# psc0628/NeRF-PRV

Hardware: AMD Instinct MI355X
Metric: ray-samples/s (field evaluations composited; candidate views rendered + scored; scene baseline, field 256^3) (higher is better)
Workload: dtype f16

## Files before the change

### nerf_prv_amd/csrc/prv_kernels.hip

```cpp
#include "prv_kernels.hpp"

#include <algorithm>

#ifndef PRV_ABLATE
#define PRV_ABLATE 0
#endif

namespace prv {


__device__ __forceinline__ void morton16(uint32_t i, uint32_t& x, uint32_t& y) {
  x = (i & 1u) | ((i >> 1) & 2u) | ((i >> 2) & 4u) | ((i >> 3) & 8u);
  y = ((i >> 1) & 1u) | ((i >> 2) & 2u) | ((i >> 3) & 4u) | ((i >> 4) & 8u);
}

constexpr float kNgpDt = 1.7320508075688772f / 1024.0f;

__device__ __forceinline__ uint32_t march_ngp(const FieldDev& fd, const float o[3], const float d[3], float t0, float t1,
                                              uint32_t (*mw)[256], int& k_lo, int& k_hi, int& first_nz, int& last_nz) {
  const float dt = kNgpDt;
  first_nz = 32;
  last_nz = -1;
  k_lo = k_hi = 0;
  float ta = t0, tb = t1;
// ... 483 lines not shown
    for (int e = 0; e < E; e++) {
      k2_lo = min(k2_lo, first_nz[e]);
      k2_hi = max(k2_hi, last_nz[e]);
    }
    uint32_t acc[E][4];
#pragma unroll
    for (int e = 0; e < E; e++)
#pragma unroll
      for (int q = 0; q < 4; q++) acc[e][q] = 0u;
    for (int k = k2_lo; k <= k2_hi; k++) {
      uint32_t w[E];
      bool behind = false;
#pragma unroll
      for (int e = 0; e < E; e++) behind = behind || (k - first_nz[e] >= kWin && k <= last_nz[e]);
      if (!((passmask >> k) & 1u)) {
#pragma unroll
        for (int e = 0; e < E; e++) w[e] = 0u;
      } else if (behind) {
        fine_word(k, w);
      } else {
#pragma unroll
        for (int e = 0; e < E; e++) {
          const int j = k - first_nz[e];
          w[e] = (j >= 0 && k <= last_nz[e]) ? mw[e][j][threadIdx.x] : 0u;
        }
      }
#pragma unroll
      for (int e = 0; e < E; e++) {
        const int j = k - first_nz[e];
        if (j < 0 || k > last_nz[e]) continue;
        const int q = j & 3;
        if (j < 4) {
#pragma unroll
          for (int u = 0; u < 4; u++)
            if (q == u) m[e][u] = w[e];
        } else {
#pragma unroll
          for (int u = 0; u < 4; u++)
            if (q == u) acc[e][u] = w[e];
          if ((q == 3 || k == last_nz[e]) && !(PRV_ABLATE & 128)) {
            const uint32_t slot = base[e] + (uint32_t)__popcll(b[e] & ((1ull << lane) - 1ull));
            P.mem[e].queue_ext[(size_t)((j >> 2) - 1) * ext_stride + slot] = make_uint4(acc[e][0], acc[e][1], acc[e][2], acc[e][3]);
#pragma unroll
            for (int u = 0; u < 4; u++) acc[e][u] = 0u;
          }
        }
      }
    }
  }
#pragma unroll
  for (int e = 0; e < E; e++) {
    const MarchSink Q{P.mem[e].queue, P.mem[e].queue_ext, ext_stride, P.mem[e].queue_count, P.mem[e].out_f32, P.mem[e].out_u8};
    march_write<true, true>(P, Q, stage, r, first_nz[e] < 32, b[e], base[e], dt, m[e], first_nz[e], last_nz[e], [](int) { return 0u; });
  }
}

__global__ __launch_bounds__(256) void occ_interleave_kernel(OccInterleaveParams P) {
  const uint32_t c = blockIdx.x * 256u + threadIdx.x;
  if (c >= P.n_cells) return;
  uint32_t v = 0u;
  for (int e = 0; e < P.n_members; e++) v |= ((P.bits[e][c >> 5] >> (c & 31u)) & 1u) << e;
  P.out[c] = (uint8_t)v;
}


__device__ __forceinline__ void clock_stamp_begin(unsigned long long* stat) {
  if (blockIdx.x == 0 && threadIdx.x == 0) {
    stat[4] = __builtin_readcyclecounter();
    stat[5] = __builtin_amdgcn_s_memrealtime();
  }
}
__device__ __forceinline__ void clock_stamp_end(unsigned long long* stat) {
  if (blockIdx.x == 0 && threadIdx.x == 0) {
    atomicAdd(stat + 2, __builtin_readcyclecounter() - stat[4]);
    atomicAdd(stat + 3, __builtin_amdgcn_s_memrealtime() - stat[5]);
  }
}

__device__ __forceinline__ int lane_id() { return (int)(threadIdx.x & 63u); }

__device__ __forceinline__ float entropy_add(float p, float H) { return p >= 1.17549435e-38f ? fmaf(p, -__builtin_amdgcn_logf(p), H) : H; }

enum : int { kRenderColour = 0, kRenderDepth = 1, kRenderEntropy = 2 };
template <int F, int NDENSE, bool NGP, bool CACHE, int MODE>
__device__ __forceinline__ void render_queue64_body(RenderParams P, const RenderDepthParams* PD, const RenderEntropyParams* PE = nullptr) {
  constexpr bool DEPTH = MODE == kRenderDepth, ENTROPY = MODE == kRenderEntropy;
  constexpr int kMoveWords = ENTROPY ? 4 : DEPTH ? 7 : 6;
  constexpr int kFrags = ENTROPY ? 8 : kNumFrags;
  __shared__ half8 wl[kFrags * 64];
  __shared__ uint32_t mv[4][32][kMoveWords];
  constexpr uint32_t kPoolCap = 192;
  __shared__ uint32_t pool[kPoolCap][kMoveWords];
  __shared__ uint32_t pool_n, pool_lock;
  for (int i = threadIdx.x; i < kFrags * 64; i += 256) wl[i] = P.field.frags64[i];
  if (threadIdx.x == 0) {
    pool_n = 0u;
    pool_lock = 0u;
  }
  __syncthreads();
  auto pool_acquire = [&]() {
    if (lane_id() == 0)
      while (atomicCAS(&pool_lock, 0u, 1u) != 0u) __builtin_amdgcn_s_sleep(2);
    __builtin_amdgcn_fence(__ATOMIC_ACQUIRE, "workgroup");
    __builtin_amdgcn_wave_barrier();
  };
  auto pool_release = [&]() {
    __builtin_amdgcn_fence(__ATOMIC_RELEASE, "workgroup");
    __builtin_amdgcn_wave_barrier();
    if (lane_id() == 0) atomicExch(&pool_lock, 0u);
  };
  const LevelDev* __restrict__ lvl = P.field.levels;
  const HashConsts hc = {P.field.hash_my_b, P.field.hash_mz_b, P.field.hash_m_b, (uint32_t)P.field.wide_offsets};

  const int lane = threadIdx.x & 63, r = lane & 31, g = lane >> 5;

  bool active = false;
  uint32_t pix = 0, rec_i = 0;
  float o[3] = {0, 0, 0}, d[3] = {0, 0, 1}, t0 = 0.f, dt = 0.f;
  uint32_t cur = 0, m1 = 0, m2 = 0, m3 = 0, base = 0;
  float T = 1.f, cr = 0.f, cg = 0.f, cb = 0.f;
  float D = 0.f;
  float Hs = 0.f;
  half8 shA = {0, 0, 0, 0, 0, 0, 0, 0}, shB = {0, 0, 0, 0, 0, 0, 0, 0};
  bool drained = false;
  unsigned long long n_eval = 0ull, n_rounds = 0ull;
  constexpr int kCached = CACHE ? 32 / F - NDENSE : 1;
  CornerCache<F> cc[kCached];
#pragma unroll
  for (int j = 0; j < kCached; j++) cc[j].key = ~0u;
  clock_stamp_begin(P.stat_evaluated);
  uint32_t q_cur = 0, q_end = 0;
  const uint32_t n_seg = (uint32_t)P.n_segments;
  const uint32_t n_sub = (uint32_t)max(P.n_sub, 1);
  uint32_t seg = n_seg > 1u ? (((uint32_t)__builtin_amdgcn_s_getreg((3 << 11) | 20) & 7u) % (n_seg / n_sub)) * n_sub + (blockIdx.x * 4u + (threadIdx.x >> 6)) % n_sub : 0u;
  uint32_t seg_tried = 0;
  const uint4* __restrict__ queue = reinterpret_cast<const uint4*>(P.queue);

  auto take_ray = [&](uint32_t ri, uint32_t next) {
    const uint4* rec = queue + (size_t)ri * kRecordWords;
    const uint4 q0 = rec[0], q1 = rec[1], q3 = rec[3];
    uint4 mk = rec[2];
    o[0] = __uint_as_float(q0.x); o[1] = __uint_as_float(q0.y); o[2] = __uint_as_float(q0.z);
    t0 = __uint_as_float(q0.w);
    d[0] = __uint_as_float(q1.x); d[1] = __uint_as_float(q1.y); d[2] = __uint_as_float(q1.z);
    dt = __uint_as_float(q1.w);
    pix = q3.x;
    rec_i = ri;
    base = 0u;
    if constexpr (NGP) {
      const uint32_t base0 = q3.y & 0xffffu;
      base = base0;
      if (next >= base0 + 128u) {
        const uint32_t j = (next - base0) >> 7;
        mk = P.queue_ext[(size_t)(j - 1u) * ((size_t)P.seg_cap * (size_t)P.n_segments) + (size_t)ri];
        base = base0 + 128u * j;
      }
    }
    cur = mk.x; m1 = mk.y; m2 = mk.z; m3 = mk.w;
    while (base + 32u <= next) {
      cur = m1; m1 = m2; m2 = m3; m3 = 0u;
      base += 32u;
    }
    if (next > base) cur &= ~0u << (next & 31u);
    while (cur == 0u && (m1 | m2 | m3) != 0u) {
      cur = m1; m1 = m2; m2 = m3; m3 = 0u;
      base += 32u;
    }
    active = true;
  };
  auto next_chunk = [&]() -> bool {
    const uint32_t info = queue[(size_t)rec_i * kRecordWords + 3].y;
    const uint32_t base0 = info & 0xffffu, n_chunks = info >> 16;
    for (uint32_t j = ((base - base0) >> 7) + 1u; j < n_chunks; j++) {
      const uint4 mk = P.queue_ext[(size_t)(j - 1u) * ((size_t)P.seg_cap * (size_t)P.n_segments) + (size_t)rec_i];
      if ((mk.x | mk.y | mk.z | mk.w) == 0u) continue;
      cur = mk.x; m1 = mk.y; m2 = mk.z; m3 = mk.w;
      base = base0 + 128u * j;
      while (cur == 0u) {
        cur = m1; m1 = m2; m2 = m3; m3 = 0u;
        base += 32u;
      }
      return true;
    }
    return false;
  };

  for (;;) {
    const bool relocate = (n_rounds & 6ull) == 0ull;
    if (relocate && !drained && P.merge_max > 0) {
      const unsigned long long act0 = __ballot(active);
      const uint32_t aA = (uint32_t)act0, aB = (uint32_t)(act0 >> 32);
      const uint32_t nA = (uint32_t)__popc(aA), nB = (uint32_t)__popc(aB);
      int src = -1;
      if (nA != 0u && nB != 0u) {
        if (nA <= (uint32_t)P.merge_max && nA <= 32u - nB) src = 0;
        else if (nB <= (uint32_t)P.merge_max && nB <= 32u - nA) src = 1;
      }
      if (src >= 0) {
        const uint32_t a_src = src == 0 ? aA : aB, a_dst = src == 0 ? aB : aA, n_src = src == 0 ? nA : nB;
        const uint32_t below = (1u << r) - 1u;
        uint32_t(*slot)[kMoveWords] = mv[threadIdx.x >> 6];
        if (g == src && active) {
          uint32_t* e = slot[__popc(a_src & below)];
          e[0] = rec_i;
          e[1] = base + (uint32_t)__builtin_ctz(cur);
          e[2] = __float_as_uint(T);
          if constexpr (ENTROPY) {
            e[3] = __float_as_uint(Hs);
          } else {
            e[3] = __float_as_uint(cr);
            e[4] = __float_as_uint(cg);
            e[5] = __float_as_uint(cb);
          }
          if constexpr (DEPTH) e[6] = __float_as_uint(D);
          active = false;
        }
        __builtin_amdgcn_fence(__ATOMIC_RELEASE, "wavefront");
        __builtin_amdgcn_wave_barrier();
        __builtin_amdgcn_fence(__ATOMIC_ACQUIRE, "wavefront");
        const uint32_t kth = (uint32_t)__popc(~a_dst & below);
        if (!((a_dst >> r) & 1u) && kth < n_src) {
          const uint32_t* e = slot[kth];
          const uint32_t ri = e[0];
          if constexpr (!ENTROPY) {
            const half8 sh = reinterpret_cast<const half8*>(queue + (size_t)ri * kRecordWords)[4 + g];
            if (src == 0) shB = sh;
            else shA = sh;
          }
          if (g != src) {
            T = __uint_as_float(e[2]);
            if constexpr (ENTROPY) {
              Hs = __uint_as_float(e[3]);
            } else {
              cr = __uint_as_float(e[3]); cg = __uint_as_float(e[4]); cb = __uint_as_float(e[5]);
            }
            if constexpr (DEPTH) D = __uint_as_float(e[6]);
            take_ray(ri, e[1]);
          }
        }
        __builtin_amdgcn_wave_barrier();
      }
    }
    if (P.pool_on && (relocate || drained)) {
      const unsigned long long act1 = __ballot(active);
      const uint32_t below = (1u << r) - 1u;
      const uint32_t in_pool = *(volatile uint32_t*)&pool_n;
#pragma unroll
      for (int grp = 0; grp < 2; grp++) {
        const uint32_t a_g = grp == 0 ? (uint32_t)act1 : (uint32_t)(act1 >> 32), n_g = (uint32_t)__popc(a_g);
        if (!drained && n_g != 0u && n_g <= (uint32_t)P.merge_max && in_pool + n_g <= kPoolCap) {
          pool_acquire();
          const uint32_t at = *(volatile uint32_t*)&pool_n;
          const bool fits = at + n_g <= kPoolCap;
          if (fits && g == grp && active) {
            uint32_t* e = pool[at + (uint32_t)__popc(a_g & below)];
            e[0] = rec_i;
            e[1] = base + (uint32_t)__builtin_ctz(cur);
            e[2] = __float_as_uint(T);
            if constexpr (ENTROPY) {
              e[3] = __float_as_uint(Hs);
            } else {
              e[3] = __float_as_uint(cr);
              e[4] = __float_as_uint(cg);
              e[5] = __float_as_uint(cb);
            }
            if constexpr (DEPTH) e[6] = __float_as_uint(D);
            active = false;
          }
          if (fits && lane == 0) *(volatile uint32_t*)&pool_n = at + n_g;
          pool_release();
        }
      }
      const unsigned long long act2 = __ballot(active);
#pragma unroll
      for (int grp = 0; grp < 2; grp++) {
        const uint32_t a_g = grp == 0 ? (uint32_t)act2 : (uint32_t)(act2 >> 32);
        const uint32_t n_idle = 32u - (uint32_t)__popc(a_g);
        if (n_idle == 0u || (a_g == 0u && !drained) || *(volatile uint32_t*)&pool_n == 0u) continue;
        pool_acquire();
        const uint32_t have = *(volatile uint32_t*)&pool_n;
        const uint32_t take = min(have, n_idle), from = have - take;
        const uint32_t kth = (uint32_t)__popc(~a_g & below);
        uint32_t ent[kMoveWords] = {};
        const bool mine = !((a_g >> r) & 1u) && kth < take;
        if (mine) {
#pragma unroll
          for (int q = 0; q < kMoveWords; q++) ent[q] = pool[from + kth][q];
        }
        if (lane == 0) *(volatile uint32_t*)&pool_n = from;
        pool_release();
        if (mine) {
          if constexpr (!ENTROPY) {
            const half8 sh = reinterpret_cast<const half8*>(queue + (size_t)ent[0] * kRecordWords)[4 + g];
            if (grp == 0) shA = sh;
            else shB = sh;
          }
          if (g == grp) {
            T = __uint_as_float(ent[2]);
            if constexpr (ENTROPY) {
              Hs = __uint_as_float(ent[3]);
            } else {
              cr = __uint_as_float(ent[3]); cg = __uint_as_float(ent[4]); cb = __uint_as_float(ent[5]);
            }
            if constexpr (DEPTH) D = __uint_as_float(ent[6]);
            take_ray(ent[0], ent[1]);
          }
        }
      }
    }
    const unsigned long long idle = __ballot(!active);
    const bool needA = (uint32_t)idle == 0xffffffffu, needB = (uint32_t)(idle >> 32) == 0xffffffffu;
    if (!drained && (needA || needB)) {
#pragma unroll
      for (int grp = 0; grp < 2; grp++) {
        if (!(grp == 0 ? needA : needB)) continue;
        while (q_cur == q_end && !drained) {
          uint32_t claim = 0;
          if (lane == 0) claim = atomicAdd(P.queue_head + 16u * seg, kClaim);
          claim = __builtin_amdgcn_readfirstlane(claim);
          const uint32_t s_lo = seg * P.seg_cap, s_cnt = min(P.queue_count[16u * seg], P.seg_cap) - P.queue_count[16u * seg + 1u];
          if (claim < s_cnt) {
            q_cur = s_lo + claim;
            q_end = min(q_cur + kClaim, s_lo + s_cnt);
          } else if (++seg_tried >= n_seg) {
            drained = true;
          } else {
            seg = seg + 1u == n_seg ? 0u : seg + 1u;
          }
        }
        const uint32_t avail = min(32u, q_end - q_cur);
        if ((uint32_t)r < avail) {
          if constexpr (!ENTROPY) {
            const half8 sh = reinterpret_cast<const half8*>(queue + (size_t)(q_cur + (uint32_t)r) * kRecordWords)[4 + g];
            if (grp == 0) shA = sh;
            else shB = sh;
          }
          if (g == grp) {
            T = 1.f; cr = 0.f; cg = 0.f; cb = 0.f;
            if constexpr (DEPTH) D = 0.f;
            if constexpr (ENTROPY) Hs = 0.f;
            take_ray(q_cur + (uint32_t)r, 0u);
          }
        }
        q_cur += avail;
      }
    }
    const unsigned long long act = __ballot(active);
    if (act == 0ull) {
      if (drained && (!P.pool_on || *(volatile uint32_t*)&pool_n == 0u)) break;
      continue;
    }
    n_eval += (unsigned long long)__popcll(act);
    n_rounds += 2ull;

    half8 f[4];
#pragma unroll
    for (int s = 0; s < 4; s++) asm volatile("" : "=v"(f[s]));
    bool last = false;
    float ts = 0.f;
    if (active) {
      const uint32_t i = base + (uint32_t)__builtin_ctz(cur);
      cur &= cur - 1u;
      if (cur == 0u) {
        last = (m1 | m2 | m3) == 0u;
        while (cur == 0u && !last) {
          cur = m1; m1 = m2; m2 = m3; m3 = 0u;
          base += 32u;
        }
        if constexpr (NGP) {
          if (last) last = !next_chunk();
        }
      }
      const float t = fmaf((float)i + 0.5f, dt, t0);
      if constexpr (DEPTH) ts = t;
      encode_sample<F, NDENSE, CACHE>(P.field.table, lvl, hc, fmaf(t, d[0], o[0]), fmaf(t, d[1], o[1]), fmaf(t, d[2], o[2]), f, cc);
    }
    swap_halves(f[0], f[1]);
    swap_halves(f[2], f[3]);
    const half8 fA[2] = {f[0], f[2]}, fB[2] = {f[1], f[3]};
    MlpOut2 mo;
    if constexpr (ENTROPY) mlp_density2(wl, lane, fA, fB, mo.densA, mo.densB);
    else mo = mlp_forward2(wl, lane, fA, fB, shA, shB);
    const float dens = g ? mo.densB[8] : mo.densA[0];
    float lr = 0.f, lg = 0.f, lb = 0.f;
    if constexpr (!ENTROPY) {
      lr = g ? mo.rgbB[8] : mo.rgbA[0];
      lg = g ? mo.rgbB[9] : mo.rgbA[1];
      lb = g ? mo.rgbB[10] : mo.rgbA[2];
    }

    bool done = false;
    if (active) {
      const float sigma = fast_exp(dens + P.field.density_bias);
      const float alpha = 1.0f - fast_exp(-(sigma * dt));
      const float wgt = alpha * T;
      if constexpr (ENTROPY) {
        Hs = entropy_add(wgt, Hs);
      } else {
        cr = fmaf(wgt, fast_sigmoid(lr), cr);
        cg = fmaf(wgt, fast_sigmoid(lg), cg);
        cb = fmaf(wgt, fast_sigmoid(lb), cb);
      }
      if constexpr (DEPTH) D = fmaf(wgt, ts, D);
      T = T * (1.0f - alpha);
      done = last || T < P.min_T;
    }
    if (done) {
      if constexpr (ENTROPY) {
        PE->out_entropy[pix] = entropy_add(T, Hs);
        PE->out_alpha[pix] = 1.0f - T;
      } else {
        const float4 v = make_float4(cr, cg, cb, 1.0f - T);
        reinterpret_cast<float4*>(P.out_f32)[pix] = v;
        if (P.last_pass && P.out_u8) P.out_u8[pix] = quantize_rgba8(v.x, v.y, v.z, v.w, P.bg);
      }
      if constexpr (DEPTH) {
        const CamDev& cam = PD->cams[PD->view_ids[(pix / PD->npix) % PD->nb]];
        const float fx = cam.c2w[2], fy = cam.c2w[6], fz = cam.c2w[10];
        const float inv = 1.0f / sqrtf(fmaf(fx, fx, fmaf(fy, fy, fz * fz)));
        PD->out_depth[pix] = D * (fmaf(d[0], fx, fmaf(d[1], fy, d[2] * fz)) * inv);
      }
      active = false;
    }
  }
  if (lane == 0 && n_eval) {
    atomicAdd(P.stat_evaluated, n_eval);
    atomicAdd(P.stat_evaluated + 1, n_rounds);
  }
  clock_stamp_end(P.stat_evaluated);
}

template <int F, int NDENSE, bool NGP, bool CACHE = false>
__global__ __launch_bounds__(256)
__attribute__((amdgpu_waves_per_eu(CACHE ? 2 : NDENSE == 0 ? 1 : 3)))
void render_queue64_kernel(RenderParams P) {
  render_queue64_body<F, NDENSE, NGP, CACHE, kRenderColour>(P, nullptr);
}

template <int F, int NDENSE, bool NGP>
__global__ __launch_bounds__(256) __attribute__((amdgpu_waves_per_eu(NDENSE == 0 ? 1 : 3)))
void render_depth_kernel(RenderDepthParams P) {
  render_queue64_body<F, NDENSE, NGP, false, kRenderDepth>(P.r, &P);
}

template <int F, int NDENSE, bool NGP>
__global__ __launch_bounds__(256) __attribute__((amdgpu_waves_per_eu(NDENSE == 0 ? 1 : 3)))
void render_entropy_kernel(RenderEntropyParams P) {
  render_queue64_body<F, NDENSE, NGP, false, kRenderEntropy>(P.r, nullptr, &P);
}


__device__ __forceinline__ int32_t first_hit_dda(const FieldDev& fd, const float o[3], const float d[3], float max_range) {
  float t0, t1;
  int32_t result = -1;
  if (ray_aabb(o, d, t0, t1)) {
    if (t1 > max_range) t1 = max_range;
    if (t1 > t0) {
      const int R = fd.occ_res;
      const float fR = (float)R;
      const float ts = t0 + 1e-6f;
      int c[3], step[3];
      float tmax[3], tdelta[3];
#pragma unroll
      for (int a = 0; a < 3; a++) {
        const float p = clamp01(fmaf(ts, d[a], o[a])) * fR;
        c[a] = min((int)p, R - 1);
        if (d[a] > 0.f) {
          step[a] = 1;
          tmax[a] = (((float)(c[a] + 1)) / fR - o[a]) / d[a];
          tdelta[a] = 1.0f / (fR * d[a]);
        } else if (d[a] < 0.f) {
          step[a] = -1;
          tmax[a] = (((float)c[a]) / fR - o[a]) / d[a];
          tdelta[a] = -1.0f / (fR * d[a]);
        } else {
          step[a] = 0;
          tmax[a] = __builtin_inff();
          tdelta[a] = __builtin_inff();
        }
      }
      for (;;) {
        const uint32_t bit = (uint32_t)c[0] + (uint32_t)R * ((uint32_t)c[1] + (uint32_t)R * (uint32_t)c[2]);
        if ((fd.occ[bit >> 5] >> (bit & 31)) & 1u) {
          result = (int32_t)bit;
          break;
        }
        const int a = tmax[0] < tmax[1] ? (tmax[0] < tmax[2] ? 0 : 2) : (tmax[1] < tmax[2] ? 1 : 2);
        const float tm = a == 0 ? tmax[0] : (a == 1 ? tmax[1] : tmax[2]);
        if (tm > t1) break;
        if (a == 0) { c[0] += step[0]; tmax[0] += tdelta[0]; if (c[0] < 0 || c[0] >= R) break; }
        else if (a == 1) { c[1] += step[1]; tmax[1] += tdelta[1]; if (c[1] < 0 || c[1] >= R) break; }
        else { c[2] += step[2]; tmax[2] += tdelta[2]; if (c[2] < 0 || c[2] >= R) break; }
      }
    }
  }
  return result;
}

__global__ __launch_bounds__(256) void first_hit_kernel(FieldDev fd, const CamDev* __restrict__ cams, int W, int H,
                                                        float max_range, int32_t* __restrict__ out) {
  const int i = blockIdx.x * 256 + threadIdx.x;
  if (i >= W * H) return;
  const int v = blockIdx.y;
  const int px = i % W, py = i / W;
  float o[3], d[3], t0, t1;
  raygen(cams[v], px, py, 0.5f, 0.5f, o, d);
  (void)t0;
  (void)t1;
  const int32_t result = first_hit_dda(fd, o, d, max_range);
  out[(size_t)v * W * H + i] = result;
}

__global__ __launch_bounds__(256) void precept_kernel(FieldDev fd, const float* __restrict__ voxels, int n, PreceptPose pose,
                                                      Rs2Intr in, float max_range, int32_t* __restrict__ out) {
  const int i = blockIdx.x * 256 + threadIdx.x;
  if (i >= n) return;
  const float origin[3] = {(float)pose.c2w[3], (float)pose.c2w[7], (float)pose.c2w[11]};
  double v[3];
#pragma unroll
// ... 496 lines not shown
}

__global__ __launch_bounds__(256) void splat_resolve_kernel(const unsigned long long* __restrict__ zbuf, int W, int H,
                                                            int flip180, uint32_t* __restrict__ out) {
  const size_t npix = (size_t)W * H;
  const size_t i = (size_t)blockIdx.x * 256 + threadIdx.x;
  if (i >= npix) return;
  const unsigned long long k = zbuf[(size_t)blockIdx.y * npix + i];
  uint32_t px = 0x00ffffffu;
  if (k != ~0ull) {
    const uint32_t col = (uint32_t)k & 0x00ffffffu;
    px = col | (col == 0x00ffffffu ? 0u : 0xff000000u);
  }
  const int x = (int)(i % W), y = (int)(i / W);
  const size_t o = flip180 ? ((size_t)(H - 1 - y) * W + (size_t)(W - 1 - x)) : i;
  out[(size_t)blockIdx.y * npix + o] = px;
}


hipError_t launch_splat_points(const float* xyz, const uint8_t* rgb, size_t n, float scale, const float off[3],
                               const CamDev* cams, int n_views, int W, int H, int point_size, int flip180,
                               unsigned long long* zbuf, uint32_t* out, hipStream_t s) {
  hipError_t e = hipMemsetAsync(zbuf, 0xff, (size_t)n_views * W * H * 8, s);
  if (e != hipSuccess) return e;
  if (n > 0)
    hipLaunchKernelGGL(splat_points_kernel, dim3((unsigned)((n + 255) / 256), n_views), dim3(256), 0, s, xyz, rgb, n, scale,
                       off[0], off[1], off[2], cams, W, H, point_size, zbuf);
  hipLaunchKernelGGL(splat_resolve_kernel, dim3((unsigned)(((size_t)W * H + 255) / 256), n_views), dim3(256), 0, s, zbuf, W, H,
                     flip180, out);
  return hipGetLastError();
}

hipError_t launch_spp_reduce(const float* stage, size_t n_pixels, int spp, const float bg[4], float* out, uint32_t* out_u8,
                             hipStream_t s) {
  unsigned blocks = (unsigned)std::min<size_t>(4096, (n_pixels + 255) / 256);
  hipLaunchKernelGGL(spp_reduce_kernel, dim3(blocks), dim3(256), 0, s, reinterpret_cast<const float4*>(stage), n_pixels, spp,
                     1.0f / (float)spp, bg[0], bg[1], bg[2], bg[3], reinterpret_cast<float4*>(out), out_u8);
  return hipGetLastError();
}

hipError_t launch_spp_reduce_depth(const float* stage, size_t n_pixels, int spp, float* out, hipStream_t s) {
  unsigned blocks = (unsigned)std::min<size_t>(4096, (n_pixels + 255) / 256);
  if (blocks == 0) return hipSuccess;
  hipLaunchKernelGGL(spp_reduce_depth_kernel, dim3(blocks), dim3(256), 0, s, stage, n_pixels, spp, 1.0f / (float)spp, out);
  return hipGetLastError();
}

hipError_t launch_march(const MarchParams& P, int n_views, int n_spp, hipStream_t s) {
  dim3 grid((unsigned)(P.live_grid ? P.live_tiles_max : P.tiles_x * P.tiles_y), (unsigned)n_views, (unsigned)(P.spp_inner_log2 > 0 ? 1 : n_spp));
  if (grid.x == 0) return hipSuccess;
  if (!P.out_f32) {
    if (P.step_mode == PRV_STEP_NGP) hipLaunchKernelGGL(march_compact_noimage_kernel<true>, grid, dim3(256), 0, s, P);
    else hipLaunchKernelGGL(march_compact_noimage_kernel<false>, grid, dim3(256), 0, s, P);
    return hipGetLastError();
  }
  if (P.step_mode == PRV_STEP_NGP) hipLaunchKernelGGL(march_compact_kernel<true>, grid, dim3(256), 0, s, P);
  else hipLaunchKernelGGL(march_compact_kernel<false>, grid, dim3(256), 0, s, P);
  return hipGetLastError();
}

hipError_t launch_occ_interleave(const OccInterleaveParams& P, hipStream_t s) {
  hipLaunchKernelGGL(occ_interleave_kernel, dim3((P.n_cells + 255u) / 256u), dim3(256), 0, s, P);
  return hipGetLastError();
}

bool march_multi_supported(int n_members) { return n_members == 2 || n_members == 5; }

hipError_t launch_march_multi(const MarchMultiParams& P, int n_views, int n_spp, hipStream_t s) {
  dim3 grid((unsigned)(P.tiles_x * P.tiles_y), (unsigned)n_views, (unsigned)(P.spp_inner_log2 > 0 ? 1 : n_spp));
  if (grid.x == 0) return hipSuccess;
  if (P.n_members == 5) hipLaunchKernelGGL((march_multi_kernel<5, 8>), grid, dim3(256), 0, s, P);
  else if (P.n_members == 2) hipLaunchKernelGGL((march_multi_kernel<2, 12>), grid, dim3(256), 0, s, P);
  else return hipErrorInvalidValue;
  return hipGetLastError();
}

int render_instance_dense_levels(const FieldDev& fd) {
  const int n = fd.n_dense_levels;
  if (!fd.hash_shared) return 0;
  if (fd.n_features == 4) return n == 5 ? 5 : n == 3 ? 3 : 0;
  return n == 10 ? 10 : n == 6 ? 6 : 0;
}

template <bool NGP>
static void launch_render_mode(const RenderParams& P, int n_blocks, hipStream_t s) {
  const int nd = render_instance_dense_levels(P.field);
  if (P.cell_cache && nd > 0) {
    if (P.field.n_features == 4 && nd == 5) {
      hipLaunchKernelGGL((render_queue64_kernel<4, 5, NGP, true>), dim3(n_blocks), dim3(256), 0, s, P);
      return;
    }
  }
  if (P.field.n_features == 4) {
    if (nd == 5) hipLaunchKernelGGL((render_queue64_kernel<4, 5, NGP>), dim3(n_blocks), dim3(256), 0, s, P);
    else if (nd == 3) hipLaunchKernelGGL((render_queue64_kernel<4, 3, NGP>), dim3(n_blocks), dim3(256), 0, s, P);
    else hipLaunchKernelGGL((render_queue64_kernel<4, 0, NGP>), dim3(n_blocks), dim3(256), 0, s, P);
  } else {
    if (nd == 10) hipLaunchKernelGGL((render_queue64_kernel<2, 10, NGP>), dim3(n_blocks), dim3(256), 0, s, P);
    else if (nd == 6) hipLaunchKernelGGL((render_queue64_kernel<2, 6, NGP>), dim3(n_blocks), dim3(256), 0, s, P);
    else hipLaunchKernelGGL((render_queue64_kernel<2, 0, NGP>), dim3(n_blocks), dim3(256), 0, s, P);
  }
}

hipError_t launch_render(const RenderParams& P, int n_blocks, hipStream_t s) {
  if (P.step_mode == PRV_STEP_NGP) launch_render_mode<true>(P, n_blocks, s);
  else launch_render_mode<false>(P, n_blocks, s);
  return hipGetLastError();
}

template <bool NGP>
static void launch_render_depth_mode(const RenderDepthParams& P, int n_blocks, hipStream_t s) {
  const int nd = render_instance_dense_levels(P.r.field);
  if (P.r.field.n_features == 4) {
    if (nd == 5) hipLaunchKernelGGL((render_depth_kernel<4, 5, NGP>), dim3(n_blocks), dim3(256), 0, s, P);
    else if (nd == 3) hipLaunchKernelGGL((render_depth_kernel<4, 3, NGP>), dim3(n_blocks), dim3(256), 0, s, P);
    else hipLaunchKernelGGL((render_depth_kernel<4, 0, NGP>), dim3(n_blocks), dim3(256), 0, s, P);
  } else {
    if (nd == 10) hipLaunchKernelGGL((render_depth_kernel<2, 10, NGP>), dim3(n_blocks), dim3(256), 0, s, P);
    else if (nd == 6) hipLaunchKernelGGL((render_depth_kernel<2, 6, NGP>), dim3(n_blocks), dim3(256), 0, s, P);
    else hipLaunchKernelGGL((render_depth_kernel<2, 0, NGP>), dim3(n_blocks), dim3(256), 0, s, P);
  }
}

hipError_t launch_render_depth(const RenderDepthParams& P, int n_blocks, hipStream_t s) {
  if (P.r.step_mode == PRV_STEP_NGP) launch_render_depth_mode<true>(P, n_blocks, s);
  else launch_render_depth_mode<false>(P, n_blocks, s);
  return hipGetLastError();
}

template <bool NGP>
static void launch_render_entropy_mode(const RenderEntropyParams& P, int n_blocks, hipStream_t s) {
  const int nd = render_instance_dense_levels(P.r.field);
  if (P.r.field.n_features == 4) {
    if (nd == 5) hipLaunchKernelGGL((render_entropy_kernel<4, 5, NGP>), dim3(n_blocks), dim3(256), 0, s, P);
    else if (nd == 3) hipLaunchKernelGGL((render_entropy_kernel<4, 3, NGP>), dim3(n_blocks), dim3(256), 0, s, P);
    else hipLaunchKernelGGL((render_entropy_kernel<4, 0, NGP>), dim3(n_blocks), dim3(256), 0, s, P);
  } else {
    if (nd == 10) hipLaunchKernelGGL((render_entropy_kernel<2, 10, NGP>), dim3(n_blocks), dim3(256), 0, s, P);
    else if (nd == 6) hipLaunchKernelGGL((render_entropy_kernel<2, 6, NGP>), dim3(n_blocks), dim3(256), 0, s, P);
    else hipLaunchKernelGGL((render_entropy_kernel<2, 0, NGP>), dim3(n_blocks), dim3(256), 0, s, P);
  }
}

hipError_t launch_render_entropy(const RenderEntropyParams& P, int n_blocks, hipStream_t s) {
  if (P.r.step_mode == PRV_STEP_NGP) launch_render_entropy_mode<true>(P, n_blocks, s);
  else launch_render_entropy_mode<false>(P, n_blocks, s);
  return hipGetLastError();
}

hipError_t launch_score_entropy(const float* entropy, const float* alpha, size_t npix, int n_views, int n_blocks, double* partial,
                                hipStream_t s) {
  hipLaunchKernelGGL(score_entropy_kernel, dim3((unsigned)n_blocks, (unsigned)n_views), dim3(256), 0, s, entropy, alpha, npix, partial);
  return hipGetLastError();
}

hipError_t launch_first_hit(const FieldDev& fd, const CamDev* cams, int n_views, int W, int H, float max_range,
                            int32_t* out, hipStream_t s) {
  dim3 grid((unsigned)((W * H + 255) / 256), (unsigned)n_views);
  hipLaunchKernelGGL(first_hit_kernel, grid, dim3(256), 0, s, fd, cams, W, H, max_range, out);
  return hipGetLastError();
}

hipError_t launch_precept(const FieldDev& fd, const float* voxels, int n, const PreceptPose& pose, const Rs2Intr& in,
                          float max_range, int32_t* out, hipStream_t s) {
  hipLaunchKernelGGL(precept_kernel, dim3((unsigned)((n + 255) / 256)), dim3(256), 0, s, fd, voxels, n, pose, in, max_range, out);
  return hipGetLastError();
}

hipError_t launch_quantize(const float* in, size_t n, const float bg[4], uint8_t* out, hipStream_t s) {
  unsigned blocks = (unsigned)((n + 255) / 256);
  if (blocks > 4096) blocks = 4096;
  if (blocks == 0) blocks = 1;
  hipLaunchKernelGGL(quantize_kernel, dim3(blocks), dim3(256), 0, s, reinterpret_cast<const float4*>(in), n,
                     bg[0], bg[1], bg[2], bg[3], reinterpret_cast<uint32_t*>(out));
  return hipGetLastError();
}

hipError_t launch_score_ensemble(const EnsembleParams& P, int method, int n_views, int n_blocks, prv_score_record* rec,
                                 hipStream_t s) {
  dim3 grid((unsigned)n_blocks, (unsigned)n_views);
  const size_t n_terms = P.pixels_per_view * (method == PRV_SCORE_ENSEMBLE_RGB ? 3 : 2);
  if (method == PRV_SCORE_ENSEMBLE_RGB)
    hipLaunchKernelGGL(score_ensemble_terms_kernel<PRV_SCORE_ENSEMBLE_RGB>, grid, dim3(256), 0, s, P);
// ... 73 lines not shown
```

Measured before the change: 24.65 billion.

## Restructure render scheduler loop to skip ballots and branchless mask advance

Restructures the persistent render loop so the active-lane ballot is carried across iterations, and the relocation, pool and refill logic only runs when it is needed (a relocate round, an idle half-wave, or drain). It makes the wave index, segment and pool count scalar via readfirstlane. It replaces the while-loop that advances occupancy mask words with a branchless select chain. It also moves the u8 output check into a template parameter. The aim is to cut per-step scheduling overhead and divergence, at the cost of more template instances and more complex control flow, where a missed ballot update could cause correctness bugs.

```diff
diff --git a/nerf_prv_amd/csrc/prv_kernels.hip b/nerf_prv_amd/csrc/prv_kernels.hip
--- a/nerf_prv_amd/csrc/prv_kernels.hip
+++ b/nerf_prv_amd/csrc/prv_kernels.hip
@@ -589,7 +589,7 @@
 __device__ __forceinline__ float entropy_add(float p, float H) { return p >= 1.17549435e-38f ? fmaf(p, -__builtin_amdgcn_logf(p), H) : H; }
 
 enum : int { kRenderColour = 0, kRenderDepth = 1, kRenderEntropy = 2 };
-template <int F, int NDENSE, bool NGP, bool CACHE, int MODE>
+template <int F, int NDENSE, bool NGP, bool CACHE, int MODE, bool U8 = false>
 __device__ __forceinline__ void render_queue64_body(RenderParams P, const RenderDepthParams* PD, const RenderEntropyParams* PE = nullptr) {
   constexpr bool DEPTH = MODE == kRenderDepth, ENTROPY = MODE == kRenderEntropy;
   constexpr int kMoveWords = ENTROPY ? 4 : DEPTH ? 7 : 6;
@@ -611,6 +611,7 @@
     __builtin_amdgcn_fence(__ATOMIC_ACQUIRE, "workgroup");
     __builtin_amdgcn_wave_barrier();
   };
+  auto pool_count = [&]() -> uint32_t { return (uint32_t)__builtin_amdgcn_readfirstlane((int)*(volatile uint32_t*)&pool_n); };
   auto pool_release = [&]() {
     __builtin_amdgcn_fence(__ATOMIC_RELEASE, "workgroup");
     __builtin_amdgcn_wave_barrier();
@@ -620,6 +621,7 @@
   const HashConsts hc = {P.field.hash_my_b, P.field.hash_mz_b, P.field.hash_m_b, (uint32_t)P.field.wide_offsets};
 
   const int lane = threadIdx.x & 63, r = lane & 31, g = lane >> 5;
+  const uint32_t wave = (uint32_t)__builtin_amdgcn_readfirstlane((int)(threadIdx.x >> 6));
 
   bool active = false;
   uint32_t pix = 0, rec_i = 0;
@@ -639,7 +641,8 @@
   uint32_t q_cur = 0, q_end = 0;
   const uint32_t n_seg = (uint32_t)P.n_segments;
   const uint32_t n_sub = (uint32_t)max(P.n_sub, 1);
-  uint32_t seg = n_seg > 1u ? (((uint32_t)__builtin_amdgcn_s_getreg((3 << 11) | 20) & 7u) % (n_seg / n_sub)) * n_sub + (blockIdx.x * 4u + (threadIdx.x >> 6)) % n_sub : 0u;
+  uint32_t seg = (uint32_t)__builtin_amdgcn_readfirstlane(
+      (int)(n_seg > 1u ? (((uint32_t)__builtin_amdgcn_s_getreg((3 << 11) | 20) & 7u) % (n_seg / n_sub)) * n_sub + (blockIdx.x * 4u + wave) % n_sub : 0u));
   uint32_t seg_tried = 0;
   const uint4* __restrict__ queue = reinterpret_cast<const uint4*>(P.queue);
 
@@ -692,170 +695,176 @@
     return false;
   };
 
+  unsigned long long act = 0ull;
   for (;;) {
-    const bool relocate = (n_rounds & 6ull) == 0ull;
-    if (relocate && !drained && P.merge_max > 0) {
-      const unsigned long long act0 = __ballot(active);
-      const uint32_t aA = (uint32_t)act0, aB = (uint32_t)(act0 >> 32);
-      const uint32_t nA = (uint32_t)__popc(aA), nB = (uint32_t)__popc(aB);
-      int src = -1;
-      if (nA != 0u && nB != 0u) {
-        if (nA <= (uint32_t)P.merge_max && nA <= 32u - nB) src = 0;
-        else if (nB <= (uint32_t)P.merge_max && nB <= 32u - nA) src = 1;
-      }
-      if (src >= 0) {
-        const uint32_t a_src = src == 0 ? aA : aB, a_dst = src == 0 ? aB : aA, n_src = src == 0 ? nA : nB;
-        const uint32_t below = (1u << r) - 1u;
-        uint32_t(*slot)[kMoveWords] = mv[threadIdx.x >> 6];
-        if (g == src && active) {
-          uint32_t* e = slot[__popc(a_src & below)];
-          e[0] = rec_i;
-          e[1] = base + (uint32_t)__builtin_ctz(cur);
-          e[2] = __float_as_uint(T);
-          if constexpr (ENTROPY) {
-            e[3] = __float_as_uint(Hs);
-          } else {
-            e[3] = __float_as_uint(cr);
-            e[4] = __float_as_uint(cg);
-            e[5] = __float_as_uint(cb);
+    for (;;) {
+      const bool relocate = (n_rounds & 6ull) == 0ull;
+      const bool group_idle = (uint32_t)act == 0u || (uint32_t)(act >> 32) == 0u;
+      if (drained ? P.pool_on != 0 : ((relocate && (P.merge_max > 0 || P.pool_on)) || group_idle)) {
+        if (relocate && !drained && P.merge_max > 0) {
+          const unsigned long long act0 = act;
+          const uint32_t aA = (uint32_t)act0, aB = (uint32_t)(act0 >> 32);
+          const uint32_t nA = (uint32_t)__popc(aA), nB = (uint32_t)__popc(aB);
+          int src = -1;
+          if (nA != 0u && nB != 0u) {
+            if (nA <= (uint32_t)P.merge_max && nA <= 32u - nB) src = 0;
+            else if (nB <= (uint32_t)P.merge_max && nB <= 32u - nA) src = 1;
           }
-          if constexpr (DEPTH) e[6] = __float_as_uint(D);
-          active = false;
-        }
-        __builtin_amdgcn_fence(__ATOMIC_RELEASE, "wavefront");
-        __builtin_amdgcn_wave_barrier();
-        __builtin_amdgcn_fence(__ATOMIC_ACQUIRE, "wavefront");
-        const uint32_t kth = (uint32_t)__popc(~a_dst & below);
-        if (!((a_dst >> r) & 1u) && kth < n_src) {
-          const uint32_t* e = slot[kth];
-          const uint32_t ri = e[0];
-          if constexpr (!ENTROPY) {
-            const half8 sh = reinterpret_cast<const half8*>(queue + (size_t)ri * kRecordWords)[4 + g];
-            if (src == 0) shB = sh;
-            else shA = sh;
-          }
-          if (g != src) {
-            T = __uint_as_float(e[2]);
-            if constexpr (ENTROPY) {
-              Hs = __uint_as_float(e[3]);
-            } else {
-              cr = __uint_as_float(e[3]); cg = __uint_as_float(e[4]); cb = __uint_as_float(e[5]);
+          if (src >= 0) {
+            const uint32_t a_src = src == 0 ? aA : aB, a_dst = src == 0 ? aB : aA, n_src = src == 0 ? nA : nB;
+            const uint32_t below = (1u << r) - 1u;
+            uint32_t(*slot)[kMoveWords] = mv[wave];
+            if (g == src && active) {
+              uint32_t* e = slot[__popc(a_src & below)];
+              e[0] = rec_i;
+              e[1] = base + (uint32_t)__builtin_ctz(cur);
+              e[2] = __float_as_uint(T);
+              if constexpr (ENTROPY) {
+                e[3] = __float_as_uint(Hs);
+              } else {
+                e[3] = __float_as_uint(cr);
+                e[4] = __float_as_uint(cg);
+                e[5] = __float_as_uint(cb);
+              }
+              if constexpr (DEPTH) e[6] = __float_as_uint(D);
+              active = false;
             }
-            if constexpr (DEPTH) D = __uint_as_float(e[6]);
-            take_ray(ri, e[1]);
+            __builtin_amdgcn_fence(__ATOMIC_RELEASE, "wavefront");
+            __builtin_amdgcn_wave_barrier();
+            __builtin_amdgcn_fence(__ATOMIC_ACQUIRE, "wavefront");
+            const uint32_t kth = (uint32_t)__popc(~a_dst & below);
+            if (!((a_dst >> r) & 1u) && kth < n_src) {
+              const uint32_t* e = slot[kth];
+              const uint32_t ri = e[0];
+              if constexpr (!ENTROPY) {
+                const half8 sh = reinterpret_cast<const half8*>(queue + (size_t)ri * kRecordWords)[4 + g];
+                if (src == 0) shB = sh;
+                else shA = sh;
+              }
+              if (g != src) {
+                T = __uint_as_float(e[2]);
+                if constexpr (ENTROPY) {
+                  Hs = __uint_as_float(e[3]);
+                } else {
+                  cr = __uint_as_float(e[3]); cg = __uint_as_float(e[4]); cb = __uint_as_float(e[5]);
+                }
+                if constexpr (DEPTH) D = __uint_as_float(e[6]);
+                take_ray(ri, e[1]);
+              }
+            }
+            __builtin_amdgcn_wave_barrier();
+            act = __ballot(active);
           }
         }
-        __builtin_amdgcn_wave_barrier();
-      }
-    }
-    if (P.pool_on && (relocate || drained)) {
-      const unsigned long long act1 = __ballot(active);
-      const uint32_t below = (1u << r) - 1u;
-      const uint32_t in_pool = *(volatile uint32_t*)&pool_n;
-#pragma unroll
-      for (int grp = 0; grp < 2; grp++) {
-        const uint32_t a_g = grp == 0 ? (uint32_t)act1 : (uint32_t)(act1 >> 32), n_g = (uint32_t)__popc(a_g);
-        if (!drained && n_g != 0u && n_g <= (uint32_t)P.merge_max && in_pool + n_g <= kPoolCap) {
-          pool_acquire();
-          const uint32_t at = *(volatile uint32_t*)&pool_n;
-          const bool fits = at + n_g <= kPoolCap;
-          if (fits && g == grp && active) {
-            uint32_t* e = pool[at + (uint32_t)__popc(a_g & below)];
-            e[0] = rec_i;
-            e[1] = base + (uint32_t)__builtin_ctz(cur);
-            e[2] = __float_as_uint(T);
-            if constexpr (ENTROPY) {
-              e[3] = __float_as_uint(Hs);
-            } else {
-              e[3] = __float_as_uint(cr);
-              e[4] = __float_as_uint(cg);
-              e[5] = __float_as_uint(cb);
+        if (P.pool_on && (relocate || drained)) {
+          const unsigned long long act1 = act;
+          const uint32_t below = (1u << r) - 1u;
+          const uint32_t in_pool = pool_count();
+#pragma unroll
+          for (int grp = 0; grp < 2; grp++) {
+            const uint32_t a_g = grp == 0 ? (uint32_t)act1 : (uint32_t)(act1 >> 32), n_g = (uint32_t)__popc(a_g);
+            if (!drained && n_g != 0u && n_g <= (uint32_t)P.merge_max && in_pool + n_g <= kPoolCap) {
+              pool_acquire();
+              const uint32_t at = pool_count();
+              const bool fits = at + n_g <= kPoolCap;
+              if (fits && g == grp && active) {
+                uint32_t* e = pool[at + (uint32_t)__popc(a_g & below)];
+                e[0] = rec_i;
+                e[1] = base + (uint32_t)__builtin_ctz(cur);
+                e[2] = __float_as_uint(T);
+                if constexpr (ENTROPY) {
+                  e[3] = __float_as_uint(Hs);
+                } else {
+                  e[3] = __float_as_uint(cr);
+                  e[4] = __float_as_uint(cg);
+                  e[5] = __float_as_uint(cb);
+                }
+                if constexpr (DEPTH) e[6] = __float_as_uint(D);
+                active = false;
+              }
+              if (fits && lane == 0) *(volatile uint32_t*)&pool_n = at + n_g;
+              pool_release();
+              act = __ballot(active);
             }
-            if constexpr (DEPTH) e[6] = __float_as_uint(D);
-            active = false;
           }
-          if (fits && lane == 0) *(volatile uint32_t*)&pool_n = at + n_g;
-          pool_release();
-        }
-      }
-      const unsigned long long act2 = __ballot(active);
-#pragma unroll
-      for (int grp = 0; grp < 2; grp++) {
-        const uint32_t a_g = grp == 0 ? (uint32_t)act2 : (uint32_t)(act2 >> 32);
-        const uint32_t n_idle = 32u - (uint32_t)__popc(a_g);
-        if (n_idle == 0u || (a_g == 0u && !drained) || *(volatile uint32_t*)&pool_n == 0u) continue;
-        pool_acquire();
-        const uint32_t have = *(volatile uint32_t*)&pool_n;
-        const uint32_t take = min(have, n_idle), from = have - take;
-        const uint32_t kth = (uint32_t)__popc(~a_g & below);
-        uint32_t ent[kMoveWords] = {};
-        const bool mine = !((a_g >> r) & 1u) && kth < take;
-        if (mine) {
-#pragma unroll
-          for (int q = 0; q < kMoveWords; q++) ent[q] = pool[from + kth][q];
-        }
-        if (lane == 0) *(volatile uint32_t*)&pool_n = from;
-        pool_release();
-        if (mine) {
-          if constexpr (!ENTROPY) {
-            const half8 sh = reinterpret_cast<const half8*>(queue + (size_t)ent[0] * kRecordWords)[4 + g];
-            if (grp == 0) shA = sh;
-            else shB = sh;
-          }
-          if (g == grp) {
-            T = __uint_as_float(ent[2]);
-            if constexpr (ENTROPY) {
-              Hs = __uint_as_float(ent[3]);
-            } else {
-              cr = __uint_as_float(ent[3]); cg = __uint_as_float(ent[4]); cb = __uint_as_float(ent[5]);
+          const unsigned long long act2 = act;
+#pragma unroll
+          for (int grp = 0; grp < 2; grp++) {
+            const uint32_t a_g = grp == 0 ? (uint32_t)act2 : (uint32_t)(act2 >> 32);
+            const uint32_t n_idle = 32u - (uint32_t)__popc(a_g);
+            if (n_idle == 0u || (a_g == 0u && !drained) || pool_count() == 0u) continue;
+            pool_acquire();
+            const uint32_t have = pool_count();
+            const uint32_t take = min(have, n_idle), from = have - take;
+            const uint32_t kth = (uint32_t)__popc(~a_g & below);
+            uint32_t ent[kMoveWords] = {};
+            const bool mine = !((a_g >> r) & 1u) && kth < take;
+            if (mine) {
+#pragma unroll
+              for (int q = 0; q < kMoveWords; q++) ent[q] = pool[from + kth][q];
             }
-            if constexpr (DEPTH) D = __uint_as_float(ent[6]);
-            take_ray(ent[0], ent[1]);
+            if (lane == 0) *(volatile uint32_t*)&pool_n = from;
+            pool_release();
+            if (mine) {
+              if constexpr (!ENTROPY) {
+                const half8 sh = reinterpret_cast<const half8*>(queue + (size_t)ent[0] * kRecordWords)[4 + g];
+                if (grp == 0) shA = sh;
+                else shB = sh;
+              }
+              if (g == grp) {
+                T = __uint_as_float(ent[2]);
+                if constexpr (ENTROPY) {
+                  Hs = __uint_as_float(ent[3]);
+                } else {
+                  cr = __uint_as_float(ent[3]); cg = __uint_as_float(ent[4]); cb = __uint_as_float(ent[5]);
+                }
+                if constexpr (DEPTH) D = __uint_as_float(ent[6]);
+                take_ray(ent[0], ent[1]);
+              }
+            }
+            act = __ballot(active);
           }
         }
-      }
-    }
-    const unsigned long long idle = __ballot(!active);
-    const bool needA = (uint32_t)idle == 0xffffffffu, needB = (uint32_t)(idle >> 32) == 0xffffffffu;
-    if (!drained && (needA || needB)) {
-#pragma unroll
-      for (int grp = 0; grp < 2; grp++) {
-        if (!(grp == 0 ? needA : needB)) continue;
-        while (q_cur == q_end && !drained) {
-          uint32_t claim = 0;
-          if (lane == 0) claim = atomicAdd(P.queue_head + 16u * seg, kClaim);
-          claim = __builtin_amdgcn_readfirstlane(claim);
-          const uint32_t s_lo = seg * P.seg_cap, s_cnt = min(P.queue_count[16u * seg], P.seg_cap) - P.queue_count[16u * seg + 1u];
-          if (claim < s_cnt) {
-            q_cur = s_lo + claim;
-            q_end = min(q_cur + kClaim, s_lo + s_cnt);
-          } else if (++seg_tried >= n_seg) {
-            drained = true;
-          } else {
-            seg = seg + 1u == n_seg ? 0u : seg + 1u;
+        const bool needA = (uint32_t)act == 0u, needB = (uint32_t)(act >> 32) == 0u;
+        if (!drained && (needA || needB)) {
+#pragma unroll
+          for (int grp = 0; grp < 2; grp++) {
+            if (!(grp == 0 ? needA : needB)) continue;
+            while (q_cur == q_end && !drained) {
+              uint32_t claim = 0;
+              if (lane == 0) claim = atomicAdd(P.queue_head + 16u * seg, kClaim);
+              claim = __builtin_amdgcn_readfirstlane(claim);
+              const uint32_t s_lo = seg * P.seg_cap, s_cnt = min(P.queue_count[16u * seg], P.seg_cap) - P.queue_count[16u * seg + 1u];
+              if (claim < s_cnt) {
+                q_cur = s_lo + claim;
+                q_end = min(q_cur + kClaim, s_lo + s_cnt);
+              } else if (++seg_tried >= n_seg) {
+                drained = true;
+              } else {
+                seg = seg + 1u == n_seg ? 0u : seg + 1u;
+              }
+            }
+            const uint32_t avail = min(32u, q_end - q_cur);
+            if ((uint32_t)r < avail) {
+              if constexpr (!ENTROPY) {
+                const half8 sh = reinterpret_cast<const half8*>(queue + (size_t)(q_cur + (uint32_t)r) * kRecordWords)[4 + g];
+                if (grp == 0) shA = sh;
+                else shB = sh;
+              }
+              if (g == grp) {
+                T = 1.f; cr = 0.f; cg = 0.f; cb = 0.f;
+                if constexpr (DEPTH) D = 0.f;
+                if constexpr (ENTROPY) Hs = 0.f;
+                take_ray(q_cur + (uint32_t)r, 0u);
+              }
+            }
+            q_cur += avail;
           }
+          act = __ballot(active);
         }
-        const uint32_t avail = min(32u, q_end - q_cur);
-        if ((uint32_t)r < avail) {
-          if constexpr (!ENTROPY) {
-            const half8 sh = reinterpret_cast<const half8*>(queue + (size_t)(q_cur + (uint32_t)r) * kRecordWords)[4 + g];
-            if (grp == 0) shA = sh;
-            else shB = sh;
-          }
-          if (g == grp) {
-            T = 1.f; cr = 0.f; cg = 0.f; cb = 0.f;
-            if constexpr (DEPTH) D = 0.f;
-            if constexpr (ENTROPY) Hs = 0.f;
-            take_ray(q_cur + (uint32_t)r, 0u);
-          }
-        }
-        q_cur += avail;
-      }
-    }
-    const unsigned long long act = __ballot(active);
-    if (act == 0ull) {
-      if (drained && (!P.pool_on || *(volatile uint32_t*)&pool_n == 0u)) break;
-      continue;
+      }
+      if (act != 0ull) break;
+      if (drained && (!P.pool_on || pool_count() == 0u)) goto finished;
     }
     n_eval += (unsigned long long)__popcll(act);
     n_rounds += 2ull;
@@ -868,15 +877,22 @@
     if (active) {
       const uint32_t i = base + (uint32_t)__builtin_ctz(cur);
       cur &= cur - 1u;
-      if (cur == 0u) {
-        last = (m1 | m2 | m3) == 0u;
-        while (cur == 0u && !last) {
-          cur = m1; m1 = m2; m2 = m3; m3 = 0u;
-          base += 32u;
-        }
-        if constexpr (NGP) {
-          if (last) last = !next_chunk();
-        }
+      last = cur == 0u && (m1 | m2 | m3) == 0u;
+      if constexpr (NGP) {
+        if (last) last = !next_chunk();
+      }
+      {
+        const bool s1 = cur == 0u, z1 = m1 == 0u, z2 = m2 == 0u;
+        const bool s2 = s1 && z1, s3 = s2 && z2;
+        const uint32_t n_cur = z1 ? (z2 ? m3 : m2) : m1;
+        const uint32_t n_m1 = s3 ? 0u : (z1 ? m3 : m2);
+        const uint32_t n_m2 = s2 ? 0u : m3;
+        const uint32_t step = z1 ? (z2 ? 96u : 64u) : 32u;
+        cur = s1 ? n_cur : cur;
+        m1 = s1 ? n_m1 : m1;
+        m2 = s1 ? n_m2 : m2;
+        m3 = s1 ? 0u : m3;
+        base += s1 ? step : 0u;
       }
       const float t = fmaf((float)i + 0.5f, dt, t0);
       if constexpr (DEPTH) ts = t;
@@ -919,7 +935,7 @@
       } else {
         const float4 v = make_float4(cr, cg, cb, 1.0f - T);
         reinterpret_cast<float4*>(P.out_f32)[pix] = v;
-        if (P.last_pass && P.out_u8) P.out_u8[pix] = quantize_rgba8(v.x, v.y, v.z, v.w, P.bg);
+        if constexpr (U8) P.out_u8[pix] = quantize_rgba8(v.x, v.y, v.z, v.w, P.bg);
       }
       if constexpr (DEPTH) {
         const CamDev& cam = PD->cams[PD->view_ids[(pix / PD->npix) % PD->nb]];
@@ -929,7 +945,9 @@
       }
       active = false;
     }
-  }
+    act = __ballot(active);
+  }
+finished:
   if (lane == 0 && n_eval) {
     atomicAdd(P.stat_evaluated, n_eval);
     atomicAdd(P.stat_evaluated + 1, n_rounds);
@@ -937,11 +955,11 @@
   clock_stamp_end(P.stat_evaluated);
 }
 
-template <int F, int NDENSE, bool NGP, bool CACHE = false>
+template <int F, int NDENSE, bool NGP, bool CACHE = false, bool U8 = false>
 __global__ __launch_bounds__(256)
 __attribute__((amdgpu_waves_per_eu(CACHE ? 2 : NDENSE == 0 ? 1 : 3)))
 void render_queue64_kernel(RenderParams P) {
-  render_queue64_body<F, NDENSE, NGP, CACHE, kRenderColour>(P, nullptr);
+  render_queue64_body<F, NDENSE, NGP, CACHE, kRenderColour, U8>(P, nullptr);
 }
 
 template <int F, int NDENSE, bool NGP>
@@ -1604,23 +1622,29 @@
   return n == 10 ? 10 : n == 6 ? 6 : 0;
 }
 
+template <int F, int NDENSE, bool NGP, bool CACHE = false>
+static void launch_colour(const RenderParams& P, int n_blocks, hipStream_t s) {
+  if (P.last_pass && P.out_u8) hipLaunchKernelGGL((render_queue64_kernel<F, NDENSE, NGP, CACHE, true>), dim3(n_blocks), dim3(256), 0, s, P);
+  else hipLaunchKernelGGL((render_queue64_kernel<F, NDENSE, NGP, CACHE, false>), dim3(n_blocks), dim3(256), 0, s, P);
+}
+
 template <bool NGP>
 static void launch_render_mode(const RenderParams& P, int n_blocks, hipStream_t s) {
   const int nd = render_instance_dense_levels(P.field);
   if (P.cell_cache && nd > 0) {
     if (P.field.n_features == 4 && nd == 5) {
-      hipLaunchKernelGGL((render_queue64_kernel<4, 5, NGP, true>), dim3(n_blocks), dim3(256), 0, s, P);
+      launch_colour<4, 5, NGP, true>(P, n_blocks, s);
       return;
     }
   }
   if (P.field.n_features == 4) {
-    if (nd == 5) hipLaunchKernelGGL((render_queue64_kernel<4, 5, NGP>), dim3(n_blocks), dim3(256), 0, s, P);
-    else if (nd == 3) hipLaunchKernelGGL((render_queue64_kernel<4, 3, NGP>), dim3(n_blocks), dim3(256), 0, s, P);
-    else hipLaunchKernelGGL((render_queue64_kernel<4, 0, NGP>), dim3(n_blocks), dim3(256), 0, s, P);
+    if (nd == 5) launch_colour<4, 5, NGP>(P, n_blocks, s);
+    else if (nd == 3) launch_colour<4, 3, NGP>(P, n_blocks, s);
+    else launch_colour<4, 0, NGP>(P, n_blocks, s);
   } else {
-    if (nd == 10) hipLaunchKernelGGL((render_queue64_kernel<2, 10, NGP>), dim3(n_blocks), dim3(256), 0, s, P);
-    else if (nd == 6) hipLaunchKernelGGL((render_queue64_kernel<2, 6, NGP>), dim3(n_blocks), dim3(256), 0, s, P);
-    else hipLaunchKernelGGL((render_queue64_kernel<2, 0, NGP>), dim3(n_blocks), dim3(256), 0, s, P);
+    if (nd == 10) launch_colour<2, 10, NGP>(P, n_blocks, s);
+    else if (nd == 6) launch_colour<2, 6, NGP>(P, n_blocks, s);
+    else launch_colour<2, 0, NGP>(P, n_blocks, s);
   }
 }
 
```

Result: no change. 24.66 billion (median of 2 runs) (+0.0%).
